# travelingspaceman/LowThrustOpt

Measured on AMD Instinct MI355X. Metric: segment-integrations/sec (state+costate+STM), higher is better.
Workload: dtype f64; 1 GPU; c2 indirect 14-dim+STM S=4096 rk4x64; segments_per_gpu=4096, global_segments=4096, kernel=pipeline8, collective=none

## Files before the change

lowthrustopt_amd/csrc/hooks/pipe_hooks.hpp:

```cpp
#pragma once
#include <hip/hip_runtime.h>

namespace lto {
namespace hook {

constexpr bool kProbeBuild = false;

struct BarrierWait {
  __device__ __forceinline__ void sync() { __syncthreads(); }
  __device__ __forceinline__ int sync_or(const int pred) { return __syncthreads_or(pred); }
  __device__ __forceinline__ void report(double*, long, int, long) const {}
  __device__ __forceinline__ void report_edges(double*, long, int, long) const {}
};
struct RegionClock {
  __device__ __forceinline__ void start() {}
  __device__ __forceinline__ void report(double*, long, int, int, long) const {}
  __device__ __forceinline__ void report_ticks(double*, long, int, long) const {}
};
struct Counter {
  __device__ __forceinline__ void bump() {}
  __device__ __forceinline__ void report(double*, long, int, long) const {}
};
struct Stamps {
  __device__ __forceinline__ void mark(int) {}
  __device__ __forceinline__ void report(double*, long, int, long) const {}
};
template <class Args>
__device__ __forceinline__ constexpr bool role_on(const Args&, int) { return true; }

}
}
```

lowthrustopt_amd/csrc/kernels_indirect_pipe32.hip:

```cpp
#include "pipe_common.hpp"

namespace lto {

constexpr int P32_SEG = 32;

template <int ND, int PM> struct Pipe32 {
  using Arg = PipeArg<ND, PM>;
  static constexpr int NI = Arg::N;
  static constexpr int NC = sizeof(typename PipeCoef<ND>::type) / sizeof(double);
  static constexpr bool LM_OFF = (ND == 14) && !Arg::LM;
  static_assert(ND == 12 || LM_OFF, "built for the laws whose RK4 stages pair");
  static constexpr int NB = LM_OFF ? ND - 1 : ND;
  static constexpr int NA = LM_OFF ? ND - 1 : ND;
  static constexpr int SD = P32_SEG * CoefBySegment::LD;
  static constexpr int NPAIR = (ND == 14) ? 4 : 3;
  static constexpr int SLABD = NPAIR * P32_SEG * 2;
  static constexpr int INT_DOUBLES = 2 * 4 * SLABD;
  static constexpr int COEF_DOUBLES = 2 * 4 * SD;
  __host__ __device__ static constexpr int lin(int e) { return (ND == 12) ? e : (e < 3 ? e : e == 3 ? 6 : e < 7 ? e - 1 : 7); }
};

typedef double p32_d2 __attribute__((ext_vector_type(2)));

template <int CTRL>
__device__ __forceinline__ double q32_from(const double x) {
  const int lo = __builtin_amdgcn_mov_dpp(__double2loint(x), CTRL, 0xF, 0xF, true);
  const int hi = __builtin_amdgcn_mov_dpp(__double2hiint(x), CTRL, 0xF, 0xF, true);
  return __hiloint2double(hi, lo);
}
__device__ __forceinline__ double q32_from_a(const double x) { return q32_from<0x00>(x); }
__device__ __forceinline__ double q32_from_b(const double x) { return q32_from<0x55>(x); }
__device__ __forceinline__ double q32_other_body(const double x) { return q32_from<0x4E>(x); }

template <int ND, int PM>
__device__ __forceinline__ void pipe32_role_base(const IndirectArgs& a, const PipeLane& L, const int seg, const int q,
                                                 double* s_int) {
  using P = Pipe32<ND, PM>;
  static_assert(ND == 12 || P::LM_OFF, "lambda_m on the chain: the stages do not pair");
  constexpr int NB = P::NB;
  constexpr bool M14 = (ND == 14);
  constexpr int V = 3, MI = 6, LR = M14 ? 7 : 6, LV = LR + 3;
  constexpr int SLAB = P::SLABD;
  const int steps = a.steps;
  const double h = L.h, h2 = 0.5 * h, h6 = h * (1.0 / 6.0), h3 = h * (1.0 / 3.0), w2 = L.w2;
  const bool is_b = (q & 1) != 0;
  const bool body2 = (q & 2) != 0;
  const double body_off = body2 ? L.tp.MU - 1.0 : L.tp.MU, body_kap = body2 ? L.tp.MU : 1.0 - L.tp.MU, body_sgn = body2 ? 1.0 : -1.0;
  auto swap_body = [](const double v) { return q32_other_body(v); };
  const double gA = is_b ? h2 : 0.0;
  const double al = is_b ? 0.0 : h2, be = is_b ? h : 0.0;
  const int own = is_b ? SLAB : 0;
  const double kt = L.tp.kappa_td;
  double y[ND];
#pragma unroll
  for (int c = 0; c < ND; ++c) y[c] = a.X[c * a.ldx + L.node];
  double inv_m = 0.0;
  if constexpr (M14) inv_m = rcp_nr(y[MI]);
  for (int step = 0; step < steps + 2; ++step) {
    if (step < steps) {
// ... 86 lines not shown
        }
        if constexpr (M14) {
          slab[2 * SLAB + 6 * P32_SEG] = y3m; slab[3 * SLAB + 6 * P32_SEG] = y4m;
          const double u4 = gf4 * im4;
          kv4[0] = __builtin_fma(w2, y4v[1], __builtin_fma(-u4, y4l[0], a4[0]));
          kv4[1] = __builtin_fma(-w2, y4v[0], __builtin_fma(-u4, y4l[1], a4[1]));
          kv4[2] = __builtin_fma(-u4, y4l[2], a4[2]);
        } else {
          kv4[0] = __builtin_fma(w2, y4v[1], a4[0]); kv4[1] = __builtin_fma(-w2, y4v[0], a4[1]); kv4[2] = a4[2];
        }
        const double kl4[3] = {__builtin_fma(w2, y4l[1], -y4g[0]), __builtin_fma(-w2, y4l[0], -y4g[1]), -y4g[2]};
#pragma unroll
        for (int i = 0; i < 3; ++i) {
          y[i] = __builtin_fma(h6, y4v[i], __builtin_fma(h3, y3v[i], ar[i]));
          y[V + i] = __builtin_fma(h6, kv4[i], __builtin_fma(h3, kv3[i], avv[i]));
          y[LR + i] = __builtin_fma(h6, g4[i], __builtin_fma(h3, g3[i], ag[i]));
          y[LV + i] = __builtin_fma(h6, kl4[i], __builtin_fma(h3, kl3[i], alv[i]));
        }
        if constexpr (M14) y[MI] = mnew;
      }
    }
    __syncthreads();
  }
  if (L.in_range && q == 0) {
    if (a.defect) {
#pragma unroll
      for (int c = 0; c < NB; ++c) a.defect[c * a.ldd + L.s] = y[c] - a.X[c * a.ldx + L.node + 1];
    }
    if (a.errors) a.errors[L.s] = 0.0;
    if (a.nacc) a.nacc[L.s] = steps;
    if (a.nrej) a.nrej[L.s] = 0;
  }
}


template <int ND, int PM>
__device__ __forceinline__ void pipe32_role_coef(const IndirectArgs& a, const PipeLane& L, const int seg, const int stage,
                                                 const double* s_int, double* s_coef, double* s_lm) {
  using P = Pipe32<ND, PM>;
  using Coef = typename PipeCoef<ND>::type;
  constexpr int NI = P::NI, NC = P::NC, SD = P::SD;
  const int steps = a.steps;
  const double as = (stage == 2) ? L.h : 0.5 * L.h;
  const double bw = (stage == 0 || stage == 3) ? L.h * (1.0 / 6.0) : L.h * (1.0 / 3.0);
  double lm_acc = 0.0;
  for (int p = 0; p < steps + 2; ++p) {
    if (p >= 1 && p <= steps) {
      const int slab = ((p - 1) & 1) * 4 + stage;
      double arg[ND], dead[ND];
#pragma unroll
      for (int c = 0; c < ND; ++c) arg[c] = 0.0;
      const p32_d2* src = reinterpret_cast<const p32_d2*>(s_int + slab * P::SLABD) + seg;
      double lv[2 * P::NPAIR];
#pragma unroll
      for (int q = 0; q < P::NPAIR; ++q) { const p32_d2 v = src[q * P32_SEG]; lv[2 * q] = v.x; lv[2 * q + 1] = v.y; }
#pragma unroll
      for (int e = 0; e < NI; ++e) arg[P::Arg::idx[e]] = lv[P::lin(e)];
      Coef vc;
      if constexpr (ND == 12) rhs12<PM, true>(arg, L.tp, dead, vc);
      else rhs14<PM, true>(arg, L.tp, dead, vc);
      if constexpr (P::LM_OFF) lm_acc = __builtin_fma(bw, dead[ND - 1], lm_acc);
      const double* o = reinterpret_cast<const double*>(&vc);
      double* dst = s_coef + slab * SD;
      constexpr int NST = P::LM_OFF ? NC - 1 : NC;
#pragma unroll
      for (int e = 0; e < NST; ++e) dst[CoefBySegment::at<P::NA>(e, seg)] = (e < 14 || e > 16) ? o[e] * as : o[e];
    }
    __syncthreads();
  }
  if constexpr (P::LM_OFF) {
    s_lm[stage * P32_SEG + seg] = lm_acc;
    __builtin_amdgcn_s_waitcnt(0xc07f);
    if (L.in_range && stage == 0 && a.defect) {
      const double sum = (s_lm[seg] + s_lm[P32_SEG + seg]) + (s_lm[2 * P32_SEG + seg] + s_lm[3 * P32_SEG + seg]);
      const long r = (long)(ND - 1) * a.ldx + L.node;
      a.defect[(ND - 1) * a.ldd + L.s] = (a.X[r] + sum) - a.X[r + 1];
    }
  }
}

template <int ND, int PM>
__device__ __forceinline__ void pipe32_role_columns(const IndirectArgs& a, const PipeLane& L, const int seg, const int col,
                                                    const double* s_coef) {
  using P = Pipe32<ND, PM>;
  constexpr int SD = P::SD, NA = P::NA;
  const int steps = a.steps;
  const ColStepConst k(L.h, L.w2);
  const double* rec = s_coef + CoefBySegment::lane_base(col, seg);
  double y[ND];
#pragma unroll
  for (int r = 0; r < ND; ++r) y[r] = (r == col) ? 1.0 : 0.0;
  for (int p = 0; p < steps + 2; ++p) {
    if (p >= 2 && col < NA) col_dpp_step<ND, SD, P::Arg::LM, NA>(rec + ((p & 1) * 4) * SD, k, p - 2, y);
    __syncthreads();
  }
  if (L.in_range && col < ND) {
    const double sc = (col < NA) ? a.stm_scale : 1.0;
    const double poison = (col < NA) ? 0.0 : L.h - L.h;
#pragma unroll
    for (int r = 0; r < ND; ++r) a.Phi[(long)(col * ND + r) * a.ldp + L.s] = __builtin_fma(y[r], sc, poison);
  }
}

template <int ND, int PM>
__global__ __launch_bounds__(768) void k_indirect_pipe32(const IndirectArgs a) {
  using P = Pipe32<ND, PM>;
  __shared__ __attribute__((aligned(16))) double s_int[P::INT_DOUBLES];
  __shared__ double s_coef[P::COEF_DOUBLES];
  __shared__ double s_lm[4 * P32_SEG];
  const int wave = __builtin_amdgcn_readfirstlane(threadIdx.x >> 6);
  const int lane = threadIdx.x & 63;
  const int seg = (wave < 2) ? wave * 16 + (lane >> 2) : (wave < 4) ? (wave - 2) * 16 + (lane & 15) : (wave - 4) * 4 + (lane >> 4);
  const PipeLane L = pipe_lane<PM, P32_SEG>(a, seg);
  if (!__syncthreads_or(L.mine)) return;
  if (wave < 2) { __builtin_amdgcn_s_setprio(3); pipe32_role_base<ND, PM>(a, L, seg, lane & 3, s_int); }
  else if (wave < 4) { __builtin_amdgcn_s_setprio(2); pipe32_role_coef<ND, PM>(a, L, seg, lane >> 4, s_int, s_coef, s_lm); }
  else pipe32_role_columns<ND, PM>(a, L, seg, lane & 15, s_coef);
}

template <int ND, int PM>
static hipError_t launch_pipe32_one(const IndirectArgs& a, hipStream_t st) {
  dim3 grid((a.S + P32_SEG - 1) / P32_SEG);
  hipLaunchKernelGGL((k_indirect_pipe32<ND, PM>), grid, dim3(768), 0, st, a);
  return hipGetLastError();
}

hipError_t launch_indirect_stm_pipe32(int ndim, int pm, const IndirectArgs& a0, hipStream_t st) {
  if (a0.S <= 0) return hipSuccess;
  if (a0.steps < 1 || !indirect_stm_pipe32_available(ndim, pm)) return hipErrorInvalidValue;
  if (ndim == 12)
    return for_classes<PM_P0, PM_P1, PM_P2, PM_PGEN>(pm, a0, [&](auto cls, const IndirectArgs& a) { return launch_pipe32_one<12, decltype(cls)::value>(a, st); });
  return for_classes<PM_P0, PM_P1>(pm, a0, [&](auto cls, const IndirectArgs& a) { return launch_pipe32_one<14, decltype(cls)::value>(a, st); });
}

}
```

lowthrustopt_amd/csrc/kernels_indirect_pipe48.hip:

```cpp
#include "pipe_common.hpp"

namespace lto {



template <int ND, int PM, int SEG_> struct Pipe48 {
  using Arg = PipeArg<ND, PM>;
  static constexpr int NI = Arg::N;
  static constexpr int NC = sizeof(typename PipeCoef<ND>::type) / sizeof(double);
  static constexpr int SEG = SEG_;
  static constexpr int SD = SEG * CoefBySegment::LD;
  static constexpr int INT_DOUBLES = 2 * 4 * NI * SEG;
  static constexpr int COEF_DOUBLES = 2 * 4 * SD;
  static constexpr bool PARK = (ND == 14) || (PM == PM_PGEN);
  static constexpr int PARK_DOUBLES = PARK ? 2 * ND * SEG : 1;
};

template <int ND, int PM, int SEG>
__device__ __forceinline__ void pipe48_role_base(const IndirectArgs& a, const PipeLane& L, const int seg, const bool live, double* s_int) {
  using P = Pipe48<ND, PM, SEG>;
  constexpr int NI = P::NI, P48_SEG = P::SEG;
  const int steps = a.steps;
  const double h = L.h, h2 = 0.5 * h, h6 = h * (1.0 / 6.0), h3 = h * (1.0 / 3.0);
  auto rhs = [&](const double (&y)[ND], double (&k)[ND]) {
    if constexpr (ND == 12) rhs12_base<PM>(y, L.tp, k);
    else rhs14_base<PM>(y, L.tp, k);
  };
  double y[ND];
#pragma unroll
  for (int c = 0; c < ND; ++c) y[c] = a.X[c * a.ldx + L.node];
  for (int p = 0; p < steps + 2; ++p) {
    if (p < steps) {
      double k[ND], yt[ND], acc[ND];
      double* slab = s_int + ((p & 1) * 4 * NI) * P48_SEG + seg;
      auto publish = [&](const int stage, const double (&arg)[ND]) {
        if (live) {
#pragma unroll
          for (int e = 0; e < NI; ++e) slab[(stage * NI + e) * P48_SEG] = arg[P::Arg::idx[e]];
        }
      };
      publish(0, y);
      rhs(y, k);
#pragma unroll
      for (int c = 0; c < ND; ++c) { acc[c] = __builtin_fma(h6, k[c], y[c]); yt[c] = __builtin_fma(h2, k[c], y[c]); }
      publish(1, yt);
      rhs(yt, k);
#pragma unroll
      for (int c = 0; c < ND; ++c) { acc[c] = __builtin_fma(h3, k[c], acc[c]); yt[c] = __builtin_fma(h2, k[c], y[c]); }
      publish(2, yt);
      rhs(yt, k);
#pragma unroll
      for (int c = 0; c < ND; ++c) { acc[c] = __builtin_fma(h3, k[c], acc[c]); yt[c] = __builtin_fma(h, k[c], y[c]); }
      publish(3, yt);
      rhs(yt, k);
#pragma unroll
      for (int c = 0; c < ND; ++c) y[c] = __builtin_fma(h6, k[c], acc[c]);
    }
    __syncthreads();
  }
  int s_e = L.s;
  long node_e = L.node;
  if constexpr (ND == 12) {
    asm volatile("" : "+v"(s_e));
    const int traj_e = s_e / a.seg_per_traj;
    node_e = (long)traj_e * a.n_nodes + (s_e - traj_e * a.seg_per_traj);
  }
  if (L.in_range && live) {
    if (a.defect) {
#pragma unroll
      for (int c = 0; c < ND; ++c) a.defect[c * a.ldd + s_e] = y[c] - a.X[c * a.ldx + node_e + 1];
    }
    if (a.errors) a.errors[s_e] = 0.0;
    if (a.nacc) a.nacc[s_e] = steps;
    if (a.nrej) a.nrej[s_e] = 0;
  }
}

template <int ND, int PM, int SEG>
__device__ __forceinline__ void pipe48_role_base_parked(const IndirectArgs& a, const PipeLane& L, const int seg, const bool live,
                                                        double* s_int, double* s_park) {
  using P = Pipe48<ND, PM, SEG>;
  constexpr int NI = P::NI, P48_SEG = P::SEG;
  const int steps = a.steps;
  const double h = L.h, h2 = 0.5 * h, h6 = h * (1.0 / 6.0), h3 = h * (1.0 / 3.0);
  auto rhs = [&](const double (&y)[ND], double (&k)[ND]) {
    if constexpr (ND == 12) rhs12_base<PM>(y, L.tp, k);
    else rhs14_base<PM>(y, L.tp, k);
  };
  int off = seg;
  asm volatile("" : "+v"(off));
  double* yw = s_park + seg;
  double* sw = s_park + ND * P48_SEG + seg;
  const double* yr = s_park + off;
  const double* sr = s_park + ND * P48_SEG + off;
  double y[ND];
#pragma unroll
  for (int c = 0; c < ND; ++c) y[c] = a.X[c * a.ldx + L.node];
  for (int p = 0; p < steps + 2; ++p) {
    if (p < steps) {
      double k[ND], yt[ND];
      double* slab = s_int + ((p & 1) * 4 * NI) * P48_SEG + seg;
      auto publish = [&](const int stage, const double (&arg)[ND]) {
        if (live) {
// ... 2 lines not shown
        }
      };
#pragma unroll
      for (int c = 0; c < ND; ++c) yw[c * P48_SEG] = y[c];
      publish(0, y);
      rhs(y, k);
#pragma unroll
      for (int c = 0; c < ND; ++c) { sw[c * P48_SEG] = __builtin_fma(h6, k[c], y[c]); yt[c] = __builtin_fma(h2, k[c], y[c]); }
      publish(1, yt);
      rhs(yt, k);
#pragma unroll
      for (int c = 0; c < ND; ++c) { sw[c * P48_SEG] = __builtin_fma(h3, k[c], sr[c * P48_SEG]); yt[c] = __builtin_fma(h2, k[c], yr[c * P48_SEG]); }
      publish(2, yt);
      rhs(yt, k);
#pragma unroll
      for (int c = 0; c < ND; ++c) { sw[c * P48_SEG] = __builtin_fma(h3, k[c], sr[c * P48_SEG]); yt[c] = __builtin_fma(h, k[c], yr[c * P48_SEG]); }
      publish(3, yt);
      rhs(yt, k);
#pragma unroll
      for (int c = 0; c < ND; ++c) y[c] = __builtin_fma(h6, k[c], sr[c * P48_SEG]);
    }
    __syncthreads();
  }
  if (L.in_range && live) {
    if (a.defect) {
#pragma unroll
      for (int c = 0; c < ND; ++c) a.defect[c * a.ldd + L.s] = y[c] - a.X[c * a.ldx + L.node + 1];
    }
    if (a.errors) a.errors[L.s] = 0.0;
    if (a.nacc) a.nacc[L.s] = steps;
    if (a.nrej) a.nrej[L.s] = 0;
  }
}

template <int ND, int PM, int SEG>
__device__ __forceinline__ void pipe48_role_coef(const IndirectArgs& a, const PipeLane& L, const int seg, const int stage,
                                                 const double* s_int, double* s_coef) {
  using P = Pipe48<ND, PM, SEG>;
  using Coef = typename PipeCoef<ND>::type;
  constexpr int NI = P::NI, NC = P::NC, P48_SEG = P::SEG;
  const int steps = a.steps;
  const double as = (stage == 2) ? L.h : 0.5 * L.h;
  for (int p = 0; p < steps + 2; ++p) {
    if (p >= 1 && p <= steps) {
      const int buf = (p - 1) & 1;
      double arg[ND], dead[ND];
#pragma unroll
      for (int c = 0; c < ND; ++c) arg[c] = 0.0;
      const double* src = s_int + ((buf * 4 + stage) * NI) * P48_SEG + seg;
#pragma unroll
      for (int e = 0; e < NI; ++e) arg[P::Arg::idx[e]] = src[e * P48_SEG];
      Coef vc;
      if constexpr (ND == 12) rhs12<PM, true>(arg, L.tp, dead, vc);
      else rhs14<PM, true>(arg, L.tp, dead, vc);
      const double* o = reinterpret_cast<const double*>(&vc);
      double* dst = s_coef + (buf * 4 + stage) * P::SD;
#pragma unroll
      for (int e = 0; e < NC; ++e) dst[CoefBySegment::at<ND>(e, seg)] = (e < 14 || e > 16) ? o[e] * as : o[e];
    }
    __syncthreads();
  }
}

template <int ND, int SEG>
__device__ __forceinline__ void pipe48_role_columns(const IndirectArgs& a, const PipeLane& L, const int seg, const int col,
                                                    const double* s_coef) {
  constexpr int SD = SEG * CoefBySegment::LD;
  const int steps = a.steps;
  const ColStepConst k(L.h, L.w2);
  double y[ND];
#pragma unroll
  for (int r = 0; r < ND; ++r) y[r] = (r == col) ? 1.0 : 0.0;
  for (int p = 0; p < steps + 2; ++p) {
    if (p >= 2 && col < ND)
      col_dpp_step<ND, SD>(s_coef + ((p & 1) * 4) * SD + CoefBySegment::lane_base(col, seg), k, p - 2, y);
    __syncthreads();
  }
  if (L.in_range && col < ND) {
#pragma unroll
    for (int r = 0; r < ND; ++r) a.Phi[(long)(col * ND + r) * a.ldp + L.s] = y[r] * a.stm_scale;
  }
}

template <int ND, int PM, int SEG>
__global__ __launch_bounds__(1024) void k_indirect_pipe48(const IndirectArgs a) {
  using P = Pipe48<ND, PM, SEG>;
  __shared__ double s_int[P::INT_DOUBLES];
  __shared__ double s_coef[P::COEF_DOUBLES];
  __shared__ double s_park[P::PARK_DOUBLES];
  const int wave = __builtin_amdgcn_readfirstlane(threadIdx.x >> 6);
  const int lane = threadIdx.x & 63;
  constexpr bool DROP12 = (SEG == 44);
  const int cj = (DROP12 && wave > 12) ? wave - 5 : wave - 4;
  const int seg_raw = (wave == 0) ? lane : (wave < 4) ? (wave - 1) * 16 + (lane & 15) : cj * 4 + (lane >> 4);
  const int seg = seg_raw < SEG ? seg_raw : SEG - 1;
  const PipeLane L = pipe_lane<PM, SEG>(a, seg);
  if (!__syncthreads_or(L.mine)) return;
  if (DROP12 && wave == 12) return;
  if (wave == 0) {
    __builtin_amdgcn_s_setprio(3);
    if constexpr (P::PARK) pipe48_role_base_parked<ND, PM, SEG>(a, L, seg, lane < SEG, s_int, s_park);
    else pipe48_role_base<ND, PM, SEG>(a, L, seg, lane < SEG, s_int);
  }
  else if (wave < 4) { __builtin_amdgcn_s_setprio(2); pipe48_role_coef<ND, PM, SEG>(a, L, seg, lane >> 4, s_int, s_coef); }
  else pipe48_role_columns<ND, SEG>(a, L, seg, lane & 15, s_coef);
}

template <int ND, int PM, int SEG>
static hipError_t launch_pipe48_one(const IndirectArgs& a, hipStream_t st) {
  dim3 grid((a.S + SEG - 1) / SEG);
  hipLaunchKernelGGL((k_indirect_pipe48<ND, PM, SEG>), grid, dim3(1024), 0, st, a);
  return hipGetLastError();
}

template <int ND, int SEG>
static hipError_t launch_pipe48_pm(int pm, const IndirectArgs& a0, hipStream_t st) {
  return for_classes<PM_P0, PM_P1, PM_P2, PM_PGEN>(pm, a0, [&](auto cls, const IndirectArgs& a) { return launch_pipe48_one<ND, decltype(cls)::value, SEG>(a, st); });
}

hipError_t launch_indirect_stm_pipe48(int ndim, int pm, const IndirectArgs& a, bool seg44, hipStream_t st) {
  if (a.S <= 0) return hipSuccess;
  if (a.steps < 1) return hipErrorInvalidValue;
  if (ndim == 12) return seg44 ? launch_pipe48_pm<12, 44>(pm, a, st) : launch_pipe48_pm<12, 48>(pm, a, st);
  if (ndim == 14) return launch_pipe48_pm<14, 48>(pm, a, st);
  return hipErrorInvalidValue;
}

}
// ... 1 lines not shown
```

lowthrustopt_amd/csrc/kernels_indirect_pipe8.hip:

```cpp
#include "pipe_common.hpp"

namespace lto {

constexpr int P8_SPIN_LIMIT = 1 << 22;

#define P8_SYNC() p8_wait.sync()
#define P8_WAIT_DECL hook::BarrierWait p8_wait
#define P8_WAIT_REPORT(a) do { if ((threadIdx.x & 63) == 0) p8_wait.report((a).defect, (a).ldd, 16, blockIdx.x * PIPE_SEG + (threadIdx.x >> 6)); } while (0)
#define P8_EDGES_REPORT(a) do { if ((threadIdx.x & 63) == 0) p8_wait.report_edges((a).defect, (a).ldd, 20, blockIdx.x * PIPE_SEG + (threadIdx.x >> 6)); } while (0)

template <int ND, int PM> struct Pipe8 {
  using Arg = PipeArg<ND, PM>;
  static constexpr int NI = Arg::N;
  static constexpr int NC = sizeof(typename PipeCoef<ND>::type) / sizeof(double);
  static constexpr int SD = CoefBySegment::stage_doubles<NC>();
  static constexpr bool LM_OFF = (ND == 14) && !Arg::LM;
  static constexpr int NB = LM_OFF ? ND - 1 : ND;
  static constexpr int NA = LM_OFF ? ND - 1 : ND;
  static constexpr int NPAIR = (ND == 14) ? 4 : 3;
  static constexpr int SLABD = NPAIR * PIPE_SEG * 2;
  static constexpr int INT_DOUBLES = 4 * 4 * SLABD;
  __host__ __device__ static constexpr int lin(int e) { return (ND == 12) ? e : (e < 3 ? e : e == 3 ? 6 : e < 7 ? e - 1 : 7); }
  __host__ __device__ static constexpr int at(int e, int seg) { return ((lin(e) >> 1) * PIPE_SEG + seg) * 2 + (lin(e) & 1); }
  static constexpr int COEF_DOUBLES = 4 * 4 * SD;
  static constexpr int HAND_DOUBLES = ND * 64;
};

// ... 1 lines not shown

struct Pipe8Flags {
  int base_steps;
  int coef_steps;
  int hand;
  int fail;
};

__device__ __forceinline__ void p8_wait_for(int* flag, const int want, int* fail) {
  int spins = 0;
  while (__hip_atomic_load(flag, __ATOMIC_ACQUIRE, __HIP_MEMORY_SCOPE_WORKGROUP) < want) {
    if (++spins >= P8_SPIN_LIMIT) { __hip_atomic_store(fail, 1, __ATOMIC_RELAXED, __HIP_MEMORY_SCOPE_WORKGROUP); break; }
    __builtin_amdgcn_s_sleep(1);
  }
}
__device__ __forceinline__ void p8_signal(int* flag, const int value) {
  asm volatile("" ::: "memory");
  if ((threadIdx.x & 63) == 0) __hip_atomic_store(flag, value, __ATOMIC_RELAXED, __HIP_MEMORY_SCOPE_WORKGROUP);
  asm volatile("" ::: "memory");
}

template <int ND, int PM>
__device__ __forceinline__ void pipe8_role_base(const IndirectArgs& a, const PipeLane& L, const int seg, const int slot,
                                                double* s_int, Pipe8Flags* fl) {
  using P = Pipe8<ND, PM>;
  constexpr int NI = P::NI, NB = P::NB;
  const int steps = a.steps, npairs = (steps + 1) >> 1;
  const double h = L.h, h2 = 0.5 * h, h6 = h * (1.0 / 6.0), h3 = h * (1.0 / 3.0);
  auto rhs = [&](const double (&y)[ND], double (&k)[ND]) {
    if constexpr (ND == 12) rhs12_base<PM>(y, L.tp, k);
    else rhs14_base<PM, !P::LM_OFF>(y, L.tp, k);
  };
  double y[ND];
#pragma unroll
  for (int c = 0; c < ND; ++c) y[c] = a.X[c * a.ldx + L.node];
  hook::RegionClock loop_clock;
  loop_clock.start();
  P8_WAIT_DECL;
  for (int p = 0; p < npairs; ++p) {
    if (PIPE_ROLE_ON(a, 1) && (PIPE_ROLE_ON(a, 16) || slot == 0)) {
      for (int j = 0; j < 2; ++j) {
        const int step = 2 * p + j;
        if (step >= steps) break;
        double k[ND], yt[ND], acc[ND], keep[NI];
#pragma unroll
        for (int c = 0; c < ND; ++c) { yt[c] = y[c]; acc[c] = y[c]; }
        auto remember = [&](int stage, const double (&arg)[ND]) {
// ... 22 lines not shown
#pragma unroll
        for (int e = 0; e < NI; ++e) dst[P::at(e, seg)] = keep[e];
        if (j == 0) p8_signal(&fl->base_steps, step + 1);
      }
    }
    P8_SYNC();
  }
  double x1[NB];
#pragma unroll
  for (int c = 0; c < NB; ++c) x1[c] = a.X[c * a.ldx + L.node + 1];
  P8_SYNC();
  P8_WAIT_REPORT(a);
  if (L.in_range && slot == 0) {
    const bool fail = fl->fail != 0;
    if (a.defect) {
#pragma unroll
      for (int c = 0; c < NB; ++c) a.defect[c * a.ldd + L.s] = fail ? __builtin_nan("") : y[c] - x1[c];
    }
    if (a.errors) a.errors[L.s] = 0.0;
    if (a.nacc) a.nacc[L.s] = steps;
    if (a.nrej) a.nrej[L.s] = 0;
    if (seg == 0) loop_clock.report(a.defect, a.ldd, 17, 18, L.s);
  }
  P8_EDGES_REPORT(a);
}

template <int CTRL>
__device__ __forceinline__ double quad_from(const double x) {
  const int lo = __builtin_amdgcn_mov_dpp(__double2loint(x), CTRL, 0xF, 0xF, true);
  const int hi = __builtin_amdgcn_mov_dpp(__double2hiint(x), CTRL, 0xF, 0xF, true);
  return __hiloint2double(hi, lo);
}
__device__ __forceinline__ double from_a(const double x) { return quad_from<0x00>(x); }
__device__ __forceinline__ double from_b(const double x) { return quad_from<0x55>(x); }
__device__ __forceinline__ double other_body(const double x) { return quad_from<0x4E>(x); }

template <int ND, int PM>
__device__ __forceinline__ void pipe8_role_base_paired(const IndirectArgs& a, const PipeLane& L, const int seg, const int q,
                                                       double* s_int, Pipe8Flags* fl) {
  using P = Pipe8<ND, PM>;
  static_assert(ND == 12 || P::LM_OFF, "lambda_m on the chain: the stages do not pair");
  constexpr int NB = P::NB;
  constexpr bool M14 = (ND == 14);
  constexpr int V = 3, MI = 6, LR = M14 ? 7 : 6, LV = LR + 3;
  constexpr int SLAB = P::SLABD;
  const int steps = a.steps;
  const double h = L.h, h2 = 0.5 * h, h6 = h * (1.0 / 6.0), h3 = h * (1.0 / 3.0), w2 = L.w2;
  const bool is_b = (q & 1) != 0;
  const bool body2 = (q & 2) != 0;
  const double body_off = body2 ? L.tp.MU - 1.0 : L.tp.MU, body_kap = body2 ? L.tp.MU : 1.0 - L.tp.MU, body_sgn = body2 ? 1.0 : -1.0;
  auto swap_body = [](const double v) { return other_body(v); };
  const double gA = is_b ? h2 : 0.0;
  const double al = is_b ? 0.0 : h2, be = is_b ? h : 0.0;
  const int own = is_b ? SLAB : 0;
  const double kt = L.tp.kappa_td;
  double y[ND];
#pragma unroll
  for (int c = 0; c < ND; ++c) y[c] = a.X[c * a.ldx + L.node];
  double inv_m = 0.0;
  if constexpr (M14) inv_m = rcp_nr(y[MI]);
  hook::RegionClock loop_clock;
  loop_clock.start();
// ... 106 lines not shown
        }
        if constexpr (M14) y[MI] = mnew;
        if (!(step & 1)) p8_signal(&fl->base_steps, step + 1);
      }
    }
    if ((step & 1) || step == steps - 1) P8_SYNC();
  }
  double x1[NB];
#pragma unroll
  for (int c = 0; c < NB; ++c) x1[c] = a.X[c * a.ldx + L.node + 1];
  P8_SYNC();
  P8_WAIT_REPORT(a);
  if (L.in_range && q == 0) {
    const bool fail = fl->fail != 0;
    if (a.defect) {
#pragma unroll
      for (int c = 0; c < NB; ++c) a.defect[c * a.ldd + L.s] = fail ? __builtin_nan("") : y[c] - x1[c];
    }
    if (a.errors) a.errors[L.s] = 0.0;
    if (a.nacc) a.nacc[L.s] = steps;
    if (a.nrej) a.nrej[L.s] = 0;
    if (seg == 0) loop_clock.report(a.defect, a.ldd, 17, 18, L.s);
  }
  P8_EDGES_REPORT(a);
}

template <int ND, int PM>
__device__ __forceinline__ void pipe8_role_coef(const IndirectArgs& a, const PipeLane& L, const int seg, const int stage,
                                                const double* s_int, double* s_coef, double* s_lm, Pipe8Flags* fl) {
  using P = Pipe8<ND, PM>;
  using Coef = typename PipeCoef<ND>::type;
  constexpr int NI = P::NI, NC = P::NC, SD = P::SD;
  const int steps = a.steps, npairs = (steps + 1) >> 1;
  const double as = (stage == 2) ? L.h : 0.5 * L.h;
  const double bw = (stage == 0 || stage == 3) ? L.h * (1.0 / 6.0) : L.h * (1.0 / 3.0);
  double lm_acc = 0.0;
  auto build = [&](const int step) {
    const int slab = (step & 3) * 4 + stage;
    double arg[ND], dead[ND];
#pragma unroll
    for (int c = 0; c < ND; ++c) arg[c] = 0.0;
    const p8_d2* src = reinterpret_cast<const p8_d2*>(s_int + slab * P::SLABD) + seg;
    double lv[2 * P::NPAIR];
#pragma unroll
    for (int q = 0; q < P::NPAIR; ++q) { const p8_d2 v = src[q * PIPE_SEG]; lv[2 * q] = v.x; lv[2 * q + 1] = v.y; }
#pragma unroll
// ... 12 lines not shown
  for (int p = 0; p < npairs + 1; ++p) {
    if (PIPE_ROLE_ON(a, 2)) {
      if (p >= 1 && 2 * p - 1 < steps) {
        build(2 * p - 1);
        p8_signal(&fl->coef_steps, 2 * p);
      }
      if (2 * p < steps) {
        if (PIPE_ROLE_ON(a, 1)) p8_wait_for(&fl->base_steps, 2 * p + 1, &fl->fail);
        build(2 * p);
      }
    }
    P8_SYNC();
  }
  P8_WAIT_REPORT(a);
  if constexpr (P::LM_OFF) {
    s_lm[stage * PIPE_SEG + seg] = lm_acc;
    __builtin_amdgcn_s_waitcnt(0xc07f);
    if (L.in_range && stage == 0 && a.defect) {
      const double sum = (s_lm[seg] + s_lm[PIPE_SEG + seg]) + (s_lm[2 * PIPE_SEG + seg] + s_lm[3 * PIPE_SEG + seg]);
      const long r = (long)(ND - 1) * a.ldx + L.node;
      a.defect[(ND - 1) * a.ldd + L.s] = fl->fail ? __builtin_nan("") : (a.X[r] + sum) - a.X[r + 1];
    }
  }
  P8_EDGES_REPORT(a);
}

template <int ND, int NA>
__device__ __forceinline__ void pipe8_store_column(const IndirectArgs& a, const PipeLane& L, const int col, const double (&y)[ND],
                                                   const bool fail) {
  if (L.in_range && col < ND) {
    const double sc = (col < NA) ? a.stm_scale : 1.0;
    const double poison = (col < NA) ? 0.0 : L.h - L.h;
#pragma unroll
    for (int r = 0; r < ND; ++r) a.Phi[(long)(col * ND + r) * a.ldp + L.s] = fail ? __builtin_nan("") : __builtin_fma(y[r], sc, poison);
  }
}

template <int ND, int PM>
__device__ __forceinline__ void pipe8_role_columns(const IndirectArgs& a, const PipeLane& L, const int seg, const int col,
                                                   const double* s_coef, Pipe8Flags* fl, const int probe_bit) {
  using P = Pipe8<ND, PM>;
  constexpr int SD = P::SD;
  const int steps = a.steps, npairs = (steps + 1) >> 1;
  const ColStepConst k(L.h, L.w2);
  const double* rec = s_coef + CoefBySegment::lane_base(col, seg);
  double y[ND];
#pragma unroll
  for (int r = 0; r < ND; ++r) y[r] = (r == col) ? 1.0 : 0.0;
  P8_WAIT_DECL;
  for (int p = 0; p < npairs + 1; ++p) {
    if (p >= 1 && PIPE_ROLE_ON(a, 4) && PIPE_ROLE_ON(a, probe_bit)) {
      const int s0 = 2 * p - 2, s1 = 2 * p - 1;
      if (col < P::NA) col_dpp_step<ND, SD, P::Arg::LM, P::NA>(rec + ((s0 & 3) * 4) * SD, k, s0, y);
      if (s1 < steps) {
        if (PIPE_ROLE_ON(a, 2)) p8_wait_for(&fl->coef_steps, s1 + 1, &fl->fail);
        if (col < P::NA) col_dpp_step<ND, SD, P::Arg::LM, P::NA>(rec + ((s1 & 3) * 4) * SD, k, s1, y);
      }
    }
    P8_SYNC();
  }
  P8_WAIT_REPORT(a);
  pipe8_store_column<ND, P::NA>(a, L, col, y, fl->fail != 0);
  P8_EDGES_REPORT(a);
}

template <int ND, int PM, bool ODD>
__device__ __forceinline__ void pipe8_role_columns_alt(const IndirectArgs& a, const PipeLane& L, const int seg, const int col,
                                                       const double* s_coef, double* s_hand, Pipe8Flags* fl) {
  using P = Pipe8<ND, PM>;
  constexpr int SD = P::SD;
  const int steps = a.steps, npairs = (steps + 1) >> 1;
  const int lane = threadIdx.x & 63;
  const ColStepConst k(L.h, L.w2);
  const double* rec = s_coef + CoefBySegment::lane_base(col, seg);
  const bool on = col < P::NA;
  double y[ND];
#pragma unroll
  for (int r = 0; r < ND; ++r) y[r] = (r == col) ? 1.0 : 0.0;
  static_assert(ND % 2 == 0, "pairs of rows");
  p8_d2* hand2 = reinterpret_cast<p8_d2*>(s_hand);
  auto load = [&]() {
    if (on) {
#pragma unroll
      for (int q = 0; q < ND / 2; ++q) { const p8_d2 v = hand2[q * 64 + lane]; y[2 * q] = v.x; y[2 * q + 1] = v.y; }
    }
  };
  auto store = [&]() {
    if (on) {
#pragma unroll
      for (int q = 0; q < ND / 2; ++q) hand2[q * 64 + lane] = p8_d2{y[2 * q], y[2 * q + 1]};
    }
// ... 1 lines not shown
  if (!ODD) __builtin_amdgcn_s_setprio(2);
  P8_WAIT_DECL;
  for (int p = 0; p < npairs + 1; ++p) {
    if (p >= 1 && PIPE_ROLE_ON(a, 4) && PIPE_ROLE_ON(a, 32)) {
      const int step = 2 * p - 2 + (ODD ? 1 : 0);
      if (!ODD) {
        if (p > 1) load();
        if (on) col_dpp_step<ND, SD, P::Arg::LM, P::NA>(rec + ((step & 3) * 4) * SD, k, step, y);
        store();
        p8_signal(&fl->hand, p);
      } else if (step < steps) {
        if (PIPE_ROLE_ON(a, 2)) p8_wait_for(&fl->coef_steps, step + 1, &fl->fail);
        p8_wait_for(&fl->hand, p, &fl->fail);
        load();
        if (on) col_dpp_step<ND, SD, P::Arg::LM, P::NA>(rec + ((step & 3) * 4) * SD, k, step, y);
        store();
      }
    }
    P8_SYNC();
  }
  P8_WAIT_REPORT(a);
  if (!ODD) {
    load();
    pipe8_store_column<ND, P::NA>(a, L, col, y, fl->fail != 0);
  }
  P8_EDGES_REPORT(a);
}

template <int ND, int PM>
__global__ __launch_bounds__(512) void k_indirect_pipe8(const IndirectArgs a) {
  using P = Pipe8<ND, PM>;
  __shared__ __attribute__((aligned(16))) double s_int[P::INT_DOUBLES];
  __shared__ double s_coef[P::COEF_DOUBLES];
  __shared__ __attribute__((aligned(16))) double s_hand[P::HAND_DOUBLES];
  __shared__ double s_lm[4 * PIPE_SEG];
  __shared__ Pipe8Flags s_fl;
  const int wave = __builtin_amdgcn_readfirstlane(threadIdx.x >> 6);
  const int lane = threadIdx.x & 63;
  const bool col_wave = (wave != 2 && wave != 3);
  const int cw = (wave == 7) ? 2 : (wave >= 4) ? 3 : wave;
  constexpr bool PAIRED = (ND == 12) || P::LM_OFF;
  const int seg = col_wave ? cw * 4 + (lane >> 4) : (PAIRED && wave == 2) ? (lane >> 2) : (lane & (PIPE_SEG - 1));
  const PipeLane L = pipe_lane<PM>(a, seg);
  if (threadIdx.x == 0) { s_fl.base_steps = 0; s_fl.coef_steps = 0; s_fl.hand = 0; s_fl.fail = 0; }
  if (!__syncthreads_or(L.mine)) return;
  if (wave == 6) return;
  if (wave == 2) {
    if constexpr (PAIRED) pipe8_role_base_paired<ND, PM>(a, L, seg, lane & 3, s_int, &s_fl);
    else pipe8_role_base<ND, PM>(a, L, seg, lane >> 4, s_int, &s_fl);
  }
  else if (wave == 3) pipe8_role_coef<ND, PM>(a, L, seg, lane >> 4, s_int, s_coef, s_lm, &s_fl);
  else if (wave == 4) pipe8_role_columns_alt<ND, PM, false>(a, L, seg, lane & 15, s_coef, s_hand, &s_fl);
  else if (wave == 5) pipe8_role_columns_alt<ND, PM, true>(a, L, seg, lane & 15, s_coef, s_hand, &s_fl);
  else pipe8_role_columns<ND, PM>(a, L, seg, lane & 15, s_coef, &s_fl, wave == 7 ? 64 : 8);
}

template <int ND, int PM>
static hipError_t launch_pipe8_one(const IndirectArgs& a, hipStream_t st) {
  dim3 grid((a.S + PIPE_SEG - 1) / PIPE_SEG);
  hipLaunchKernelGGL((k_indirect_pipe8<ND, PM>), grid, dim3(512), 0, st, a);
  return hipGetLastError();
}

template <int ND>
static hipError_t launch_pipe8_pm(int pm, const IndirectArgs& a0, hipStream_t st) {
  return for_classes<PM_P0, PM_P1, PM_P2, PM_PGEN>(pm, a0, [&](auto cls, const IndirectArgs& a) { return launch_pipe8_one<ND, decltype(cls)::value>(a, st); });
}

hipError_t launch_indirect_stm_pipe8(int ndim, int pm, const IndirectArgs& a, hipStream_t st) {
  if (a.S <= 0) return hipSuccess;
  if (a.steps < 1) return hipErrorInvalidValue;
  if (ndim == 12) return launch_pipe8_pm<12>(pm, a, st);
  if (ndim == 14) return launch_pipe8_pm<14>(pm, a, st);
  return hipErrorInvalidValue;
}

}
// ... 1 lines not shown
```

lowthrustopt_amd/csrc/pipe_common.hpp:

```cpp
#pragma once
#include "kernels.hpp"
#include <pipe_hooks.hpp>

namespace lto {

constexpr int PIPE_SEG = 16;

template <int ND> struct PipeCoef { using type = VarCoef12; };
template <> struct PipeCoef<14> { using type = VarCoef14; };
template <int ND, int PM> struct PipeArg {
  static constexpr bool LM = false;
  static constexpr int N = 6;
  static constexpr int idx[6] = {0, 1, 2, 9, 10, 11};
  using Coef = VarCoef12;
};
template <int PM> struct PipeArg<14, PM> {
  static constexpr bool LM = !(PM == PM_P0 || PM == PM_P1);
  static constexpr int N = LM ? 8 : 7;
  static constexpr int idx[8] = {0, 1, 2, 6, 10, 11, 12, 13};
  using Coef = VarCoef14;
};

struct CoefBySegment {
  static constexpr int LD = 33;
// ... 8 lines not shown
  long node;
  bool in_range;
  bool mine;
  double h, w2;
  TrajParams tp;
};

template <int PM, int SEGS = PIPE_SEG>
__device__ __forceinline__ PipeLane pipe_lane(const IndirectArgs& a, const int seg) {
  PipeLane L;
  const int s_raw = blockIdx.x * SEGS + seg;
  const int s_lin = s_raw < a.S ? s_raw : a.S - 1;
  L.s = a.order ? a.order[s_lin] : s_lin;
  const int traj = L.s / a.seg_per_traj;
  const int i = L.s - traj * a.seg_per_traj;
  L.node = (long)traj * a.n_nodes + i;
  const long tg = (long)traj * a.t_stride + i;
  L.tp = a.tp[(long)traj * a.tp_stride];
  L.h = (a.t[tg + 1] - a.t[tg]) / (double)a.steps;
  L.w2 = 2.0 * L.tp.omega;
  L.mine = !a.class_filter || p_class(L.tp.p) == PM;
  L.in_range = (s_raw < a.S) && L.mine;
  return L;
}

#define PIPE_ROLE_ON(a, bit) hook::role_on((a), (bit))

template <int N>
__device__ __forceinline__ void fmac_b(double& acc, const double c, const double x) {
  asm("v_fmac_f64_dpp %0, %1, %2 row_newbcast:%3 row_mask:0xf bank_mask:0xf" : "+v"(acc) : "v"(c), "v"(x), "n"(N));
}
template <int N>
__device__ __forceinline__ void fmac_bn(double& acc, const double c, const double x) {
  asm("v_fmac_f64_dpp %0, -%1, %2 row_newbcast:%3 row_mask:0xf bank_mask:0xf" : "+v"(acc) : "v"(c), "v"(x), "n"(N));
}

template <int NA, int E, bool NEG = false>
__device__ __forceinline__ void fmac_c(double& acc, const double cA, const double cB, const double x) {
  static_assert(E < 2 * NA && NA <= 16, "record value outside the active lanes");
  if constexpr (E < NA) { if constexpr (NEG) fmac_bn<E>(acc, cA, x); else fmac_b<E>(acc, cA, x); }
  else { if constexpr (NEG) fmac_bn<E - NA>(acc, cB, x); else fmac_b<E - NA>(acc, cB, x); }
}

template <int ND, bool LM = true, int NA = ND>
__device__ __forceinline__ void col_dpp_stage(const double cA, const double cB, const double aw2, const double a,
                                              const double (&arg)[ND], const double (&init)[ND], double (&out)[ND]) {
// ... 65 lines not shown
```

Before: 59.63 million segment-integrations/s.

## Stage Phi output through LDS and write rows coalesced across all waves

Result: faster. 60.30 million segment-integrations/s (median of 6 runs) (+1.1%).

```diff
diff --git a/lowthrustopt_amd/csrc/hooks/pipe_hooks.hpp b/lowthrustopt_amd/csrc/hooks/pipe_hooks.hpp
--- a/lowthrustopt_amd/csrc/hooks/pipe_hooks.hpp
+++ b/lowthrustopt_amd/csrc/hooks/pipe_hooks.hpp
@@ -9,6 +9,8 @@
 struct BarrierWait {
   __device__ __forceinline__ void sync() { __syncthreads(); }
   __device__ __forceinline__ int sync_or(const int pred) { return __syncthreads_or(pred); }
+  __device__ __forceinline__ void stamp(int) {}
+  __device__ __forceinline__ void drained() {}
   __device__ __forceinline__ void report(double*, long, int, long) const {}
   __device__ __forceinline__ void report_edges(double*, long, int, long) const {}
 };
diff --git a/lowthrustopt_amd/csrc/kernels_indirect_pipe32.hip b/lowthrustopt_amd/csrc/kernels_indirect_pipe32.hip
--- a/lowthrustopt_amd/csrc/kernels_indirect_pipe32.hip
+++ b/lowthrustopt_amd/csrc/kernels_indirect_pipe32.hip
@@ -3,6 +3,7 @@
 namespace lto {
 
 constexpr int P32_SEG = 32;
+constexpr int P32_WAVES = 12;
 
 template <int ND, int PM> struct Pipe32 {
   using Arg = PipeArg<ND, PM>;
@@ -34,7 +35,7 @@
 
 template <int ND, int PM>
 __device__ __forceinline__ void pipe32_role_base(const IndirectArgs& a, const PipeLane& L, const int seg, const int q,
-                                                 double* s_int) {
+                                                 double* s_int, const double* s_coef, const int wave) {
   using P = Pipe32<ND, PM>;
   static_assert(ND == 12 || P::LM_OFF, "lambda_m on the chain: the stages do not pair");
   constexpr int NB = P::NB;
@@ -167,21 +168,24 @@
     }
     __syncthreads();
   }
+  long node_e = L.node;
+  asm volatile("" : "+v"(node_e));
   if (L.in_range && q == 0) {
     if (a.defect) {
 #pragma unroll
-      for (int c = 0; c < NB; ++c) a.defect[c * a.ldd + L.s] = y[c] - a.X[c * a.ldx + L.node + 1];
+      for (int c = 0; c < NB; ++c) a.defect[c * a.ldd + L.s] = y[c] - a.X[c * a.ldx + node_e + 1];
     }
     if (a.errors) a.errors[L.s] = 0.0;
     if (a.nacc) a.nacc[L.s] = steps;
     if (a.nrej) a.nrej[L.s] = 0;
   }
+  pipe_store_phi<ND, P32_SEG, P32_WAVES>(a, s_coef, wave);
 }
 
 
 template <int ND, int PM>
 __device__ __forceinline__ void pipe32_role_coef(const IndirectArgs& a, const PipeLane& L, const int seg, const int stage,
-                                                 const double* s_int, double* s_coef, double* s_lm) {
+                                                 const double* s_int, double* s_coef, double* s_lm, const int wave) {
   using P = Pipe32<ND, PM>;
   using Coef = typename PipeCoef<ND>::type;
   constexpr int NI = P::NI, NC = P::NC, SD = P::SD;
@@ -222,11 +226,12 @@
       a.defect[(ND - 1) * a.ldd + L.s] = (a.X[r] + sum) - a.X[r + 1];
     }
   }
+  pipe_store_phi<ND, P32_SEG, P32_WAVES>(a, s_coef, wave);
 }
 
 template <int ND, int PM>
 __device__ __forceinline__ void pipe32_role_columns(const IndirectArgs& a, const PipeLane& L, const int seg, const int col,
-                                                    const double* s_coef) {
+                                                    double* s_coef, const int wave) {
   using P = Pipe32<ND, PM>;
   constexpr int SD = P::SD, NA = P::NA;
   const int steps = a.steps;
@@ -239,12 +244,12 @@
     if (p >= 2 && col < NA) col_dpp_step<ND, SD, P::Arg::LM, NA>(rec + ((p & 1) * 4) * SD, k, p - 2, y);
     __syncthreads();
   }
-  if (L.in_range && col < ND) {
-    const double sc = (col < NA) ? a.stm_scale : 1.0;
-    const double poison = (col < NA) ? 0.0 : L.h - L.h;
-#pragma unroll
-    for (int r = 0; r < ND; ++r) a.Phi[(long)(col * ND + r) * a.ldp + L.s] = __builtin_fma(y[r], sc, poison);
-  }
+  const double sc = (col < NA) ? a.stm_scale : 1.0;
+  const double poison = (col < NA) ? 0.0 : L.h - L.h;
+  double v[ND];
+#pragma unroll
+  for (int r = 0; r < ND; ++r) v[r] = __builtin_fma(y[r], sc, poison);
+  pipe_store_phi<ND, P32_SEG, P32_WAVES>(a, s_coef, wave, true, L, seg, col, v);
 }
 
 template <int ND, int PM>
@@ -258,9 +263,9 @@
   const int seg = (wave < 2) ? wave * 16 + (lane >> 2) : (wave < 4) ? (wave - 2) * 16 + (lane & 15) : (wave - 4) * 4 + (lane >> 4);
   const PipeLane L = pipe_lane<PM, P32_SEG>(a, seg);
   if (!__syncthreads_or(L.mine)) return;
-  if (wave < 2) { __builtin_amdgcn_s_setprio(3); pipe32_role_base<ND, PM>(a, L, seg, lane & 3, s_int); }
-  else if (wave < 4) { __builtin_amdgcn_s_setprio(2); pipe32_role_coef<ND, PM>(a, L, seg, lane >> 4, s_int, s_coef, s_lm); }
-  else pipe32_role_columns<ND, PM>(a, L, seg, lane & 15, s_coef);
+  if (wave < 2) { __builtin_amdgcn_s_setprio(3); pipe32_role_base<ND, PM>(a, L, seg, lane & 3, s_int, s_coef, wave); }
+  else if (wave < 4) { __builtin_amdgcn_s_setprio(2); pipe32_role_coef<ND, PM>(a, L, seg, lane >> 4, s_int, s_coef, s_lm, wave); }
+  else pipe32_role_columns<ND, PM>(a, L, seg, lane & 15, s_coef, wave);
 }
 
 template <int ND, int PM>
diff --git a/lowthrustopt_amd/csrc/kernels_indirect_pipe48.hip b/lowthrustopt_amd/csrc/kernels_indirect_pipe48.hip
--- a/lowthrustopt_amd/csrc/kernels_indirect_pipe48.hip
+++ b/lowthrustopt_amd/csrc/kernels_indirect_pipe48.hip
@@ -14,10 +14,13 @@
   static constexpr int COEF_DOUBLES = 2 * 4 * SD;
   static constexpr bool PARK = (ND == 14) || (PM == PM_PGEN);
   static constexpr int PARK_DOUBLES = PARK ? 2 * ND * SEG : 1;
+  static constexpr int STORE_WAVES = (SEG == 44) ? 15 : 16;
+  static_assert(PhiTile<ND, SEG>::DOUBLES <= COEF_DOUBLES, "the Phi tile lives in the coefficient ring");
 };
 
 template <int ND, int PM, int SEG>
-__device__ __forceinline__ void pipe48_role_base(const IndirectArgs& a, const PipeLane& L, const int seg, const bool live, double* s_int) {
+__device__ __forceinline__ void pipe48_role_base(const IndirectArgs& a, const PipeLane& L, const int seg, const bool live, double* s_int,
+                                                 const double* s_coef) {
   using P = Pipe48<ND, PM, SEG>;
   constexpr int NI = P::NI, P48_SEG = P::SEG;
   const int steps = a.steps;
@@ -62,8 +65,10 @@
   long node_e = L.node;
   if constexpr (ND == 12) {
     asm volatile("" : "+v"(s_e));
-    const int traj_e = s_e / a.seg_per_traj;
-    node_e = (long)traj_e * a.n_nodes + (s_e - traj_e * a.seg_per_traj);
+    int spt_e = a.seg_per_traj;
+    asm volatile("" : "+s"(spt_e));
+    const int traj_e = s_e / spt_e;
+    node_e = (long)traj_e * a.n_nodes + (s_e - traj_e * spt_e);
   }
   if (L.in_range && live) {
     if (a.defect) {
@@ -74,11 +79,12 @@
     if (a.nacc) a.nacc[s_e] = steps;
     if (a.nrej) a.nrej[s_e] = 0;
   }
+  pipe_store_phi<ND, SEG, P::STORE_WAVES>(a, s_coef, 0);
 }
 
 template <int ND, int PM, int SEG>
 __device__ __forceinline__ void pipe48_role_base_parked(const IndirectArgs& a, const PipeLane& L, const int seg, const bool live,
-                                                        double* s_int, double* s_park) {
+                                                        double* s_int, double* s_park, const double* s_coef) {
   using P = Pipe48<ND, PM, SEG>;
   constexpr int NI = P::NI, P48_SEG = P::SEG;
   const int steps = a.steps;
@@ -127,20 +133,23 @@
     }
     __syncthreads();
   }
+  long node_e = L.node;
+  asm volatile("" : "+v"(node_e));
   if (L.in_range && live) {
     if (a.defect) {
 #pragma unroll
-      for (int c = 0; c < ND; ++c) a.defect[c * a.ldd + L.s] = y[c] - a.X[c * a.ldx + L.node + 1];
+      for (int c = 0; c < ND; ++c) a.defect[c * a.ldd + L.s] = y[c] - a.X[c * a.ldx + node_e + 1];
     }
     if (a.errors) a.errors[L.s] = 0.0;
     if (a.nacc) a.nacc[L.s] = steps;
     if (a.nrej) a.nrej[L.s] = 0;
   }
+  pipe_store_phi<ND, SEG, P::STORE_WAVES>(a, s_coef, 0);
 }
 
 template <int ND, int PM, int SEG>
 __device__ __forceinline__ void pipe48_role_coef(const IndirectArgs& a, const PipeLane& L, const int seg, const int stage,
-                                                 const double* s_int, double* s_coef) {
+                                                 const double* s_int, double* s_coef, const int rank) {
   using P = Pipe48<ND, PM, SEG>;
   using Coef = typename PipeCoef<ND>::type;
   constexpr int NI = P::NI, NC = P::NC, P48_SEG = P::SEG;
@@ -165,11 +174,12 @@
     }
     __syncthreads();
   }
-}
-
-template <int ND, int SEG>
+  pipe_store_phi<ND, SEG, P::STORE_WAVES>(a, s_coef, rank);
+}
+
+template <int ND, int SEG, int NW>
 __device__ __forceinline__ void pipe48_role_columns(const IndirectArgs& a, const PipeLane& L, const int seg, const int col,
-                                                    const double* s_coef) {
+                                                    double* s_coef, const int rank) {
   constexpr int SD = SEG * CoefBySegment::LD;
   const int steps = a.steps;
   const ColStepConst k(L.h, L.w2);
@@ -181,10 +191,10 @@
       col_dpp_step<ND, SD>(s_coef + ((p & 1) * 4) * SD + CoefBySegment::lane_base(col, seg), k, p - 2, y);
     __syncthreads();
   }
-  if (L.in_range && col < ND) {
-#pragma unroll
-    for (int r = 0; r < ND; ++r) a.Phi[(long)(col * ND + r) * a.ldp + L.s] = y[r] * a.stm_scale;
-  }
+  double v[ND];
+#pragma unroll
+  for (int r = 0; r < ND; ++r) v[r] = y[r] * a.stm_scale;
+  pipe_store_phi<ND, SEG, NW>(a, s_coef, rank, true, L, seg, col, v);
 }
 
 template <int ND, int PM, int SEG>
@@ -202,13 +212,14 @@
   const PipeLane L = pipe_lane<PM, SEG>(a, seg);
   if (!__syncthreads_or(L.mine)) return;
   if (DROP12 && wave == 12) return;
+  const int rank = (DROP12 && wave > 12) ? wave - 1 : wave;
   if (wave == 0) {
     __builtin_amdgcn_s_setprio(3);
-    if constexpr (P::PARK) pipe48_role_base_parked<ND, PM, SEG>(a, L, seg, lane < SEG, s_int, s_park);
-    else pipe48_role_base<ND, PM, SEG>(a, L, seg, lane < SEG, s_int);
-  }
-  else if (wave < 4) { __builtin_amdgcn_s_setprio(2); pipe48_role_coef<ND, PM, SEG>(a, L, seg, lane >> 4, s_int, s_coef); }
-  else pipe48_role_columns<ND, SEG>(a, L, seg, lane & 15, s_coef);
+    if constexpr (P::PARK) pipe48_role_base_parked<ND, PM, SEG>(a, L, seg, lane < SEG, s_int, s_park, s_coef);
+    else pipe48_role_base<ND, PM, SEG>(a, L, seg, lane < SEG, s_int, s_coef);
+  }
+  else if (wave < 4) { __builtin_amdgcn_s_setprio(2); pipe48_role_coef<ND, PM, SEG>(a, L, seg, lane >> 4, s_int, s_coef, rank); }
+  else pipe48_role_columns<ND, SEG, P::STORE_WAVES>(a, L, seg, lane & 15, s_coef, rank);
 }
 
 template <int ND, int PM, int SEG>
diff --git a/lowthrustopt_amd/csrc/kernels_indirect_pipe8.hip b/lowthrustopt_amd/csrc/kernels_indirect_pipe8.hip
--- a/lowthrustopt_amd/csrc/kernels_indirect_pipe8.hip
+++ b/lowthrustopt_amd/csrc/kernels_indirect_pipe8.hip
@@ -3,6 +3,10 @@
 namespace lto {
 
 constexpr int P8_SPIN_LIMIT = 1 << 22;
+
+constexpr int P8_STORE_WAVES = 7;
+constexpr int P8_BASE_RANK = 2, P8_COEF_RANK = 3;
+__device__ __forceinline__ int p8_store_rank(const int wave) { return wave < 6 ? wave : 6; }
 
 #define P8_SYNC() p8_wait.sync()
 #define P8_WAIT_DECL hook::BarrierWait p8_wait
@@ -50,7 +54,7 @@
 
 template <int ND, int PM>
 __device__ __forceinline__ void pipe8_role_base(const IndirectArgs& a, const PipeLane& L, const int seg, const int slot,
-                                                double* s_int, Pipe8Flags* fl) {
+                                                double* s_int, const double* s_coef, Pipe8Flags* fl) {
   using P = Pipe8<ND, PM>;
   constexpr int NI = P::NI, NB = P::NB;
   const int steps = a.steps, npairs = (steps + 1) >> 1;
@@ -119,6 +123,7 @@
     if (a.nrej) a.nrej[L.s] = 0;
     if (seg == 0) loop_clock.report(a.defect, a.ldd, 17, 18, L.s);
   }
+  pipe_store_phi<ND, PIPE_SEG, P8_STORE_WAVES>(a, s_coef, P8_BASE_RANK);
   P8_EDGES_REPORT(a);
 }
 
@@ -134,7 +139,7 @@
 
 template <int ND, int PM>
 __device__ __forceinline__ void pipe8_role_base_paired(const IndirectArgs& a, const PipeLane& L, const int seg, const int q,
-                                                       double* s_int, Pipe8Flags* fl) {
+                                                       double* s_int, const double* s_coef, Pipe8Flags* fl) {
   using P = Pipe8<ND, PM>;
   static_assert(ND == 12 || P::LM_OFF, "lambda_m on the chain: the stages do not pair");
   constexpr int NB = P::NB;
@@ -287,6 +292,7 @@
     if (a.nrej) a.nrej[L.s] = 0;
     if (seg == 0) loop_clock.report(a.defect, a.ldd, 17, 18, L.s);
   }
+  pipe_store_phi<ND, PIPE_SEG, P8_STORE_WAVES>(a, s_coef, P8_BASE_RANK);
   P8_EDGES_REPORT(a);
 }
 
@@ -345,23 +351,27 @@
       a.defect[(ND - 1) * a.ldd + L.s] = fl->fail ? __builtin_nan("") : (a.X[r] + sum) - a.X[r + 1];
     }
   }
+  pipe_store_phi<ND, PIPE_SEG, P8_STORE_WAVES>(a, s_coef, P8_COEF_RANK);
   P8_EDGES_REPORT(a);
 }
 
-template <int ND, int NA>
-__device__ __forceinline__ void pipe8_store_column(const IndirectArgs& a, const PipeLane& L, const int col, const double (&y)[ND],
-                                                   const bool fail) {
-  if (L.in_range && col < ND) {
-    const double sc = (col < NA) ? a.stm_scale : 1.0;
-    const double poison = (col < NA) ? 0.0 : L.h - L.h;
-#pragma unroll
-    for (int r = 0; r < ND; ++r) a.Phi[(long)(col * ND + r) * a.ldp + L.s] = fail ? __builtin_nan("") : __builtin_fma(y[r], sc, poison);
-  }
+template <int ND, int NA, class Wait>
+__device__ __forceinline__ void pipe8_store_column(const IndirectArgs& a, const PipeLane& L, const int seg, const int col, const double (&y)[ND],
+                                                   const bool fail, double* s_coef, const int wave, Wait& w) {
+  const double sc = (col < NA) ? a.stm_scale : 1.0;
+  const double poison = (col < NA) ? 0.0 : L.h - L.h;
+  double v[ND];
+#pragma unroll
+  for (int r = 0; r < ND; ++r) v[r] = fail ? __builtin_nan("") : __builtin_fma(y[r], sc, poison);
+  w.stamp(0);
+  pipe_store_phi<ND, PIPE_SEG, P8_STORE_WAVES>(a, s_coef, p8_store_rank(wave), true, L, seg, col, v);
+  w.stamp(1);
+  w.drained();
 }
 
 template <int ND, int PM>
 __device__ __forceinline__ void pipe8_role_columns(const IndirectArgs& a, const PipeLane& L, const int seg, const int col,
-                                                   const double* s_coef, Pipe8Flags* fl, const int probe_bit) {
+                                                   double* s_coef, Pipe8Flags* fl, const int wave) {
   using P = Pipe8<ND, PM>;
   constexpr int SD = P::SD;
   const int steps = a.steps, npairs = (steps + 1) >> 1;
@@ -372,7 +382,7 @@
   for (int r = 0; r < ND; ++r) y[r] = (r == col) ? 1.0 : 0.0;
   P8_WAIT_DECL;
   for (int p = 0; p < npairs + 1; ++p) {
-    if (p >= 1 && PIPE_ROLE_ON(a, 4) && PIPE_ROLE_ON(a, probe_bit)) {
+    if (p >= 1 && PIPE_ROLE_ON(a, 4) && PIPE_ROLE_ON(a, wave == 7 ? 64 : 8)) {
       const int s0 = 2 * p - 2, s1 = 2 * p - 1;
       if (col < P::NA) col_dpp_step<ND, SD, P::Arg::LM, P::NA>(rec + ((s0 & 3) * 4) * SD, k, s0, y);
       if (s1 < steps) {
@@ -383,13 +393,13 @@
     P8_SYNC();
   }
   P8_WAIT_REPORT(a);
-  pipe8_store_column<ND, P::NA>(a, L, col, y, fl->fail != 0);
+  pipe8_store_column<ND, P::NA>(a, L, seg, col, y, fl->fail != 0, s_coef, wave, p8_wait);
   P8_EDGES_REPORT(a);
 }
 
 template <int ND, int PM, bool ODD>
 __device__ __forceinline__ void pipe8_role_columns_alt(const IndirectArgs& a, const PipeLane& L, const int seg, const int col,
-                                                       const double* s_coef, double* s_hand, Pipe8Flags* fl) {
+                                                       double* s_coef, double* s_hand, Pipe8Flags* fl) {
   using P = Pipe8<ND, PM>;
   constexpr int SD = P::SD;
   const int steps = a.steps, npairs = (steps + 1) >> 1;
@@ -437,7 +447,12 @@
   P8_WAIT_REPORT(a);
   if (!ODD) {
     load();
-    pipe8_store_column<ND, P::NA>(a, L, col, y, fl->fail != 0);
+    pipe8_store_column<ND, P::NA>(a, L, seg, col, y, fl->fail != 0, s_coef, 4, p8_wait);
+  } else {
+    p8_wait.stamp(0);
+    pipe_store_phi<ND, PIPE_SEG, P8_STORE_WAVES>(a, s_coef, p8_store_rank(5));
+    p8_wait.stamp(1);
+    p8_wait.drained();
   }
   P8_EDGES_REPORT(a);
 }
@@ -461,13 +476,13 @@
   if (!__syncthreads_or(L.mine)) return;
   if (wave == 6) return;
   if (wave == 2) {
-    if constexpr (PAIRED) pipe8_role_base_paired<ND, PM>(a, L, seg, lane & 3, s_int, &s_fl);
-    else pipe8_role_base<ND, PM>(a, L, seg, lane >> 4, s_int, &s_fl);
+    if constexpr (PAIRED) pipe8_role_base_paired<ND, PM>(a, L, seg, lane & 3, s_int, s_coef, &s_fl);
+    else pipe8_role_base<ND, PM>(a, L, seg, lane >> 4, s_int, s_coef, &s_fl);
   }
   else if (wave == 3) pipe8_role_coef<ND, PM>(a, L, seg, lane >> 4, s_int, s_coef, s_lm, &s_fl);
   else if (wave == 4) pipe8_role_columns_alt<ND, PM, false>(a, L, seg, lane & 15, s_coef, s_hand, &s_fl);
   else if (wave == 5) pipe8_role_columns_alt<ND, PM, true>(a, L, seg, lane & 15, s_coef, s_hand, &s_fl);
-  else pipe8_role_columns<ND, PM>(a, L, seg, lane & 15, s_coef, &s_fl, wave == 7 ? 64 : 8);
+  else pipe8_role_columns<ND, PM>(a, L, seg, lane & 15, s_coef, &s_fl, wave);
 }
 
 template <int ND, int PM>
diff --git a/lowthrustopt_amd/csrc/pipe_common.hpp b/lowthrustopt_amd/csrc/pipe_common.hpp
--- a/lowthrustopt_amd/csrc/pipe_common.hpp
+++ b/lowthrustopt_amd/csrc/pipe_common.hpp
@@ -54,6 +54,60 @@
   L.mine = !a.class_filter || p_class(L.tp.p) == PM;
   L.in_range = (s_raw < a.S) && L.mine;
   return L;
+}
+
+template <int ND, int SEGS> struct PhiTile {
+  static constexpr int RPI = SEGS <= 16 ? 4 : SEGS <= 32 ? 2 : 1;
+  static constexpr int LPR = 64 / RPI;
+  static constexpr int GROUPS = ND * ND / RPI;
+  static constexpr int CS = ND * SEGS + 1;
+  static constexpr int TABLE = ND * CS;
+  static constexpr int DOUBLES = TABLE + (SEGS + 1) / 2;
+  static_assert(SEGS <= LPR && (ND * ND) % RPI == 0 && ND % 2 == 0 && CS % 2 == 1, "row groups / bank arithmetic above");
+  __host__ __device__ static constexpr int at(int col, int row, int seg) { return col * CS + row * SEGS + seg; }
+};
+
+template <int ND, int SEGS>
+__device__ __forceinline__ void pipe_phi_put(double* ring, const PipeLane& L, const int seg, const int col, const double (&v)[ND]) {
+  using T = PhiTile<ND, SEGS>;
+  if (col < ND) {
+#pragma unroll
+    for (int r = 0; r < ND; ++r) ring[T::at(col, r, seg)] = v[r];
+  }
+  if (col == 0) reinterpret_cast<int*>(ring + T::TABLE)[seg] = L.in_range ? L.s : -1;
+}
+
+template <int ND, int SEGS, int NW>
+__device__ __forceinline__ void pipe_phi_rows(const IndirectArgs& a, const double* ring, const int rank) {
+  using T = PhiTile<ND, SEGS>;
+  int lane = threadIdx.x & 63;
+  asm volatile("" : "+v"(lane));
+  const int sub = lane / T::LPR, seg = lane % T::LPR;
+  const int tgt = (seg < SEGS) ? reinterpret_cast<const int*>(ring + T::TABLE)[seg] : -1;
+  double* dst = a.Phi + ((long)(rank * T::RPI + sub) * a.ldp + tgt);
+  const long stride = (long)(NW * T::RPI) * a.ldp;
+#pragma unroll
+  for (int i = 0; i < (T::GROUPS + NW - 1) / NW; ++i) {
+    const int g = rank + i * NW;
+    if (g < T::GROUPS && tgt >= 0) {
+      const int row = g * T::RPI + sub;
+      __builtin_nontemporal_store(ring[T::at(row / ND, row % ND, seg)], dst + i * stride);
+    }
+  }
+}
+
+template <int ND, int SEGS, int NW>
+__device__ __forceinline__ void pipe_store_phi(const IndirectArgs& a, double* ring, const int rank, const bool put, const PipeLane& L,
+                                               const int seg, const int col, const double (&v)[ND]) {
+  if (put) pipe_phi_put<ND, SEGS>(ring, L, seg, col, v);
+  __syncthreads();
+  pipe_phi_rows<ND, SEGS, NW>(a, ring, rank);
+}
+
+template <int ND, int SEGS, int NW>
+__device__ __forceinline__ void pipe_store_phi(const IndirectArgs& a, const double* ring, const int rank) {
+  __syncthreads();
+  pipe_phi_rows<ND, SEGS, NW>(a, ring, rank);
 }
 
 #define PIPE_ROLE_ON(a, bit) hook::role_on((a), (bit))
```
